# mandyxmq/NeuralBTF-tiny-cuda-nn

Hardware: AMD Instinct MI355X
Metric: training steps/sec at batch=2^18, config_hash.json (HashGrid+64-wide MLP) (higher is better)
Workload: dtype fp16 storage / fp32 MFMA accumulate; 1 GPU; HashGrid L16 F2 log2T15 s1.5 base16 + FullyFusedMLP W64 H2 ReLU, RelativeL2, Adam, B=2^18; global_batch=262144, per_gpu_batch=262144, parallelism=dp1

## Files before the change

neuralbtf-tiny-cuda-nn_amd/csrc/capi.cpp:

```cpp
#include "../../include/tcnn_mi355x.h"
#include "debug_api.h"
#include "debug_grid_bwd.h"

#include <algorithm>
#include <cmath>
#include <cstring>
#include <limits>
#include <mutex>

#include "loss_device.h"
#include "loss_torch.h"
#include "optimizers.h"
#include "runtime.h"

using namespace tcnn_amd;

namespace {
thread_local std::string g_last_error;
thread_local std::string g_str;

std::mutex g_log_mutex;
tcnn_log_callback_t g_log_cb = nullptr;
void* g_log_user = nullptr;

// ... 677 lines not shown
	return guard([&] {
		t->t->require_plain_adam("The data-parallel peer exchange");
		t->t->dp_peer_attach(blobs);
	});
}
int tcnn_trainer_dp_peer_detach(tcnn_trainer* t) {
	return guard([&] { t->t->dp_peer_detach(); });
}
int tcnn_trainer_dp_peer_set_timeout(tcnn_trainer* t, double seconds) {
	return guard([&] { t->t->dp_peer_set_timeout(seconds); });
}
int tcnn_debug_peer_loopback(tcnn_trainer* t, int nranks) {
	return guard([&] {
		t->t->require_plain_adam("The data-parallel peer exchange");
		t->t->dp_peer_loopback(nranks);
	});
}
int tcnn_trainer_dp_peer_abandon(tcnn_trainer* t) {
	return guard([&] { t->t->dp_peer_abandon(); });
}
int tcnn_trainer_dp_gather_state(tcnn_trainer* t, void* stream) {
	return guard([&] { t->t->dp_gather_state((hipStream_t)stream); });
}
float tcnn_trainer_loss(tcnn_trainer* t, void* stream) {
	float v = -1.0f;
	if (guard([&] { v = t->t->loss((hipStream_t)stream); }) != 0) return -1.0f;
	return v;
}
int tcnn_trainer_loss_value(tcnn_trainer* t, void* stream, float* out) {
	return guard([&] {
// ... 101 lines not shown
	return guard([&] {
		TCNN_CHECK(name && ptr, "optimizer_buffer: null name or result pointer");
		*ptr = t->t->optimizer_buffer(name, elem_bytes);
	});
}
int tcnn_trainer_learning_rate(const tcnn_trainer* t, float* learning_rate) {
	return guard([&] {
		TCNN_CHECK(learning_rate != nullptr, "learning_rate: null result pointer");
		*learning_rate = t->t->learning_rate();
	});
}
const char* tcnn_trainer_optimizer_schedule(const tcnn_trainer* t) { return !t->t->opt ? "adam" : t->t->opt_inline ? "inline" : "staged"; }
int tcnn_trainer_set_learning_rate(tcnn_trainer* t, float learning_rate) {
	return guard([&] { t->t->set_learning_rate(learning_rate); });
}
void* tcnn_trainer_param_gradients(tcnn_trainer* t) { return t->t->g16.p; }
float* tcnn_trainer_gradients_fp32(tcnn_trainer* t) { return t->t->g32.as<float>(); }
int tcnn_trainer_optimizer_state(tcnn_trainer* t, float** m1, float** m2, uint32_t** steps) {
	if (m1) *m1 = t->t->m1.as<float>();
	if (m2) *m2 = t->t->m2.as<float>();
	if (steps) *steps = t->t->steps.as<uint32_t>();
	return 0;
}
int tcnn_trainer_set_gradient_scale(tcnn_trainer* t, float s) {
	TrainerHost& h = *t->t;
	h.grad_scale_user = s;
	h.grad_scale = s / (float)h.dp_nranks();
	return 0;
}
int tcnn_trainer_set_loss_scale(tcnn_trainer* t, float loss_scale) {
	return guard([&] {
		TCNN_CHECK(loss_scale > 0.0f && std::isfinite(loss_scale), "set_loss_scale: the loss scale must be positive and finite");
		t->t->loss_scale = loss_scale;
// ... 183 lines not shown
```

neuralbtf-tiny-cuda-nn_amd/csrc/dp.cpp:

```cpp
#include <dlfcn.h>

#include <rccl/rccl.h>

#include <cstring>
#include <mutex>

#include "runtime.h"

namespace tcnn_amd {

namespace {
struct RcclApi {
	decltype(&ncclGetUniqueId) get_unique_id = nullptr;
	decltype(&ncclCommInitRank) comm_init_rank = nullptr;
	decltype(&ncclCommDestroy) comm_destroy = nullptr;
	decltype(&ncclAllReduce) all_reduce = nullptr;
	decltype(&ncclReduceScatter) reduce_scatter = nullptr;
	decltype(&ncclAllGather) all_gather = nullptr;
	decltype(&ncclGetErrorString) error_string = nullptr;
};

const RcclApi& rccl() {
	static std::once_flag once;
	static RcclApi api;
// ... 67 lines not shown
}

static void grow_preserve(DevBuf& b, size_t bytes, size_t valid) {
	if (b.bytes >= bytes) return;
	DevBuf n;
	n.reserve(bytes);
	TCNN_HIP_CHECK(hipMemset(n.p, 0, bytes));
	if (b.p && valid) TCNN_HIP_CHECK(hipMemcpy(n.p, b.p, valid, hipMemcpyDeviceToDevice));
	std::swap(b.p, n.p);
	std::swap(b.bytes, n.bytes);
}

void TrainerHost::set_dp(DpComm* c, bool sharded) {
	TCNN_CHECK(!peer_attached, "set_dp: the trainer is attached to a peer exchange (detach it first)");
	if (dp && dp_sharded && dp_state_partial) dp_gather_state(nullptr);
	TCNN_HIP_CHECK(hipDeviceSynchronize());
	dp = c;
	dp_sharded = c && sharded;
	dp_state_partial = false;
	grad_scale = grad_scale_user / (float)dp_nranks();
	if (graph) set_graph(use_graph);
	if (!dp_sharded) return;
	const uint64_t N = (uint64_t)c->nranks;
	dp_per = (n_params + N - 1) / N;
	const size_t pad = (size_t)(dp_per * N);
	grow_preserve(w32, pad * 4, n_params * 4);
	grow_preserve(w16, pad * 2, n_params * 2);
	grow_preserve(g16, pad * 2, n_params * 2);
	grow_preserve(g32, pad * 4, n_params * 4);
	grow_preserve(m1, pad * 4, n_params * 4);
// ... 35 lines not shown
		optimizer_step_range(st, lo, hi);
		c.all_gather(w16.p, (size_t)dp_per, 2, st);
		dp_state_partial = true;
	} else {
		optimizer_step(st);
	}
	timer.mark(st, 3);
}

void TrainerHost::dp_gather_state(hipStream_t st) {
	if (peer_attached) {
		if (dp_state_partial) dp_peer_gather_state(st);
		return;
	}
	if (!dp || !dp_sharded || !dp_state_partial) return;
	for (DevBuf* b : {&w32, &m1, &m2, &steps}) dp->all_gather(b->p, (size_t)dp_per, 4, st);
	TCNN_HIP_CHECK(hipStreamSynchronize(st));
	dp_state_partial = false;
}

}
```

neuralbtf-tiny-cuda-nn_amd/csrc/dp_peer.hip:

```cpp
#include <cstdlib>
#include <cstring>
#include <vector>

#include "adam_device.h"
#include "runtime.h"

namespace tcnn_amd {

namespace {

constexpr uint32_t PEER_MAGIC = 0x50454552u;
constexpr int PEER_MAX_RANKS = 64;
constexpr int PEER_NBUF = 4;
enum PeerBuf { PB_G32 = 0, PB_W16, PB_STATE, PB_FLAGS };
enum PeerSlot { SLOT_GRAD = 0, SLOT_WEIGHTS = 1, SLOT_GATHER = 2, SLOT_DETACH = 3, SLOT_PROBE = 4 };
constexpr int PROBE_WORD = 16;

__host__ __device__ inline uint32_t probe_token(int rank) { return PEER_MAGIC ^ (0x9e3779b9u * (uint32_t)(rank + 1)); }
enum PeerCtr { CTR_STEP = 0, CTR_SYNC = 1, CTR_ERR = 2, CTR_ARRIVE = 3 };

struct PeerBlob {
	uint32_t magic, nranks, rank, device;
	uint64_t n_params, per;
	uint64_t pci;
// ... 247 lines not shown
static void grow_keep(DevBuf& b, size_t bytes, size_t valid) {
	if (b.bytes >= bytes) return;
	DevBuf n;
	n.reserve(bytes);
	TCNN_HIP_CHECK(hipMemset(n.p, 0, bytes));
	if (b.p && valid) TCNN_HIP_CHECK(hipMemcpy(n.p, b.p, valid, hipMemcpyDeviceToDevice));
	std::swap(b.p, n.p);
	std::swap(b.bytes, n.bytes);
}

void TrainerHost::dp_peer_export(int nranks, int rank, void* blob_out) {
	TCNN_CHECK(!dp, "peer exchange: detach the RCCL communicator first (set_dp(NULL))");
	TCNN_CHECK(nranks >= 1 && rank >= 0 && rank < nranks, "peer exchange: rank outside [0, nranks)");
	TCNN_CHECK(nranks <= PEER_MAX_RANKS, "peer exchange: at most 64 ranks (the ranks of one node)");
	if (peer) dp_peer_detach();
	TCNN_HIP_CHECK(hipDeviceSynchronize());
	auto pd = std::make_shared<PeerDp>();
	pd->nranks = nranks;
	pd->rank = rank;
	const uint64_t per = ((n_params + nranks - 1) / nranks + 7) / 8 * 8;
	pd->per = per;
	const size_t pad = (size_t)(per * nranks);
	grow_keep(w32, pad * 4, n_params * 4);
	grow_keep(w16, pad * 2, n_params * 2);
	grow_keep(g16, pad * 2, n_params * 2);
	grow_keep(g32, pad * 4, n_params * 4);
	grow_keep(m1, pad * 4, n_params * 4);
	grow_keep(m2, pad * 4, n_params * 4);
	grow_keep(steps, pad * 4, n_params * 4);
	const size_t xbytes[PEER_NBUF] = {pad * 4, pad * 2, 4 * pad * 4, 256};
// ... 218 lines not shown
```

neuralbtf-tiny-cuda-nn_amd/csrc/kernels.h:

```cpp
#pragma once

#include "common.h"

namespace tcnn_amd {

struct LevelInfo;

struct GridCall {
	uint32_t D, F, L;
	HashType hash;
	bool hash_grid;
	Interp interp;
	const LevelInfo* levels;
	GridOpts opts;
};

struct GridSlice {
	uint32_t level;
	uint32_t begin;
	uint32_t end;
	uint32_t f0;
	uint32_t nf;
};

// ... 42 lines not shown
}

struct AdamArgs {
	uint32_t n, n_matrix;
	float loss_scale, grad_scale;
	float lr, beta1, beta2, eps, l2_reg, rel_decay, abs_decay, clip, nonmat_lr_factor;
	float lower_lr_bound, upper_lr_bound;
	int opt_matrix, opt_nonmatrix;
	float inv_loss_scale;
	uint32_t begin;
	const float* part;
	uint32_t n_parts, part_stride;
	const float* factor_table;
	uint32_t factor_n;
	const GridSlabMap* part_map;
};

struct AdamBuffers {
	float* w32;
	_Float16* w16;
	float* g32;
	_Float16* g16;
	float* m1;
	float* m2;
	uint32_t* steps;
};

struct GradFinalize {
	void* out = nullptr;
	float s = 1.0f;
	int out_f32 = 0;
// ... 116 lines not shown
	int dldenc_pairs;
	float* wgrad_partial;
	float* loss_partial;
};
void launch_mlp_tile_train(hipStream_t st, uint32_t W, uint32_t IN, uint32_t NH, int act, TileTrainArgs a);
bool tile_infer_supported(uint32_t W, uint32_t IN, uint32_t NH, uint32_t outp, int act);
uint32_t tile_infer_blocks(uint32_t B, uint32_t W, uint32_t IN, uint32_t NH);
void launch_mlp_tile_infer(hipStream_t st, uint32_t W, uint32_t IN, uint32_t NH, int act, int out_act, uint32_t B, const void* params16,
                           const void* enc16, void* out16);

void launch_generate_uniform(hipStream_t st, uint64_t n, uint64_t state, uint64_t inc, float* out, float lo, float hi);
void launch_generate_logistic(hipStream_t st, uint64_t n, uint64_t state, uint64_t inc, float* out, float mean, float stddev);
void launch_add_perturbation(hipStream_t st, uint32_t n, const void* out16, const float* noise, void* pert16);
void launch_adam(hipStream_t st, const AdamArgs& a, float* w32, void* w16, const float* grad32, void* grad16,
                 float* m1, float* m2, uint32_t* steps);

void launch_cast_f32_f16(hipStream_t st, const float* in, void* out, size_t n);
void launch_cast_f16_f32(hipStream_t st, const void* in, float* out, size_t n);
void launch_scale_f16(hipStream_t st, const void* in, void* out, float s, size_t n);
void launch_div_f32(hipStream_t st, float* x, float s, size_t n);
void launch_scale_f32(hipStream_t st, const float* in, float* out, float s, size_t n);
void launch_div_f16(hipStream_t st, const void* in, void* out, float s, size_t n, bool out_f32);
void launch_grad_finalize(hipStream_t st, const float* g, void* out, float s, size_t n, bool out_f32);

void launch_relative_l2(hipStream_t st, uint32_t B, uint32_t stride, uint32_t dims, float loss_scale,
                        const void* pred16, const float* target, float* values, void* grads16);

void launch_sum(hipStream_t st, const float* in, uint32_t n, float* out);

bool layered_width_supported(uint32_t w);
// ... 81 lines not shown
```

neuralbtf-tiny-cuda-nn_amd/csrc/kernels.hip:

```cpp
#include "kernels.h"

#include <cstdlib>

#include "adam_device.h"
#include "grid_device.h"
#include "mlp_fused.h"

namespace tcnn_amd {

__global__ __launch_bounds__(256) void k_reduce_groups(const float* __restrict__ in, uint32_t n_parts, uint32_t group,
                                                        uint32_t stride, uint32_t n, float* __restrict__ out, uint32_t out_stride) {
	const uint32_t p4 = (blockIdx.x * blockDim.x + threadIdx.x) * 4;
	if (p4 >= n) return;
	const uint32_t j0 = blockIdx.y * group;
	const uint32_t j1 = min(n_parts, j0 + group);
	float* dst = out + (size_t)blockIdx.y * out_stride;
	if (p4 + 4 <= n && (stride % 4) == 0 && (out_stride % 4) == 0) {
		f4 s = {0.0f, 0.0f, 0.0f, 0.0f};
		s = slab_sum((const f4*)(in + (size_t)j0 * stride + p4), stride / 4, j1 - j0);
		*(f4*)(dst + p4) = s;
	} else {
		for (uint32_t p = p4; p < n && p < p4 + 4; ++p) {
			float s = 0.0f;
			s = slab_sum(in + (size_t)j0 * stride + p, stride, j1 - j0);
// ... 137 lines not shown
}
void launch_add_perturbation(hipStream_t st, uint32_t n, const void* out16, const float* noise, void* pert16) {
	if (!n) return;
	hipLaunchKernelGGL(k_add_perturbation, dim3(div_round_up(n, 256u)), dim3(256), 0, st, n, (const _Float16*)out16, noise, (_Float16*)pert16);
	TCNN_HIP_CHECK(hipGetLastError());
}

void launch_generate_uniform(hipStream_t st, uint64_t n, uint64_t state, uint64_t inc, float* out, float lo, float hi) {
	if (n == 0) return;
	const uint64_t n_thr = (n + 3) / 4;
	hipLaunchKernelGGL(k_generate_uniform, dim3((uint32_t)((n_thr + 127) / 128)), dim3(128), 0, st, n, state, inc, out, lo, hi - lo);
	TCNN_HIP_CHECK(hipGetLastError());
}


__global__ __launch_bounds__(256) void k_adam(const AdamArgs a, float* __restrict__ w32, _Float16* __restrict__ w16,
                                               const float* __restrict__ grad32, _Float16* __restrict__ grad16,
                                               float* __restrict__ m1, float* __restrict__ m2, uint32_t* __restrict__ steps) {
	const uint32_t i = a.begin + blockIdx.x * blockDim.x + threadIdx.x;
	if (i >= a.n) return;
	float gsum;
	if (a.part) {
		const uint32_t q = a.part_map ? grid_slab_index(a.part_map, i - a.begin) : i - a.begin;
		gsum = slab_sum(a.part + q, a.part_stride, a.n_parts);
		((float*)grad32)[i] = gsum;
	} else {
		gsum = grad32[i];
	}
	const AdamBuffers s{w32, w16, (float*)grad32, grad16, m1, m2, steps};
	adam_update(a, s, i, gsum);
}

void launch_adam(hipStream_t st, const AdamArgs& a, float* w32, void* w16, const float* grad32, void* grad16,
                 float* m1, float* m2, uint32_t* steps) {
	if (a.n <= a.begin) return;
	hipLaunchKernelGGL(k_adam, dim3(div_round_up(a.n - a.begin, 256)), dim3(256), 0, st, a, w32, (_Float16*)w16, grad32, (_Float16*)grad16, m1, m2, steps);
	TCNN_HIP_CHECK(hipGetLastError());
}

__global__ void k_cast_f32_f16(const float* __restrict__ in, _Float16* __restrict__ out, size_t n) {
	const size_t i = (size_t)blockIdx.x * blockDim.x + threadIdx.x;
	if (i < n) out[i] = (_Float16)in[i];
}
__global__ void k_cast_f16_f32(const _Float16* __restrict__ in, float* __restrict__ out, size_t n) {
	const size_t i = (size_t)blockIdx.x * blockDim.x + threadIdx.x;
	if (i < n) out[i] = (float)in[i];
}
__global__ void k_scale_f16(const _Float16* __restrict__ in, _Float16* __restrict__ out, float s, size_t n) {
	const size_t i = (size_t)blockIdx.x * blockDim.x + threadIdx.x;
	if (i < n) out[i] = f16_rn((float)in[i] * s);
}
// ... 149 lines not shown
```

neuralbtf-tiny-cuda-nn_amd/csrc/runtime.cpp:

```cpp
#include "runtime.h"
#include "loss_device.h"

#include <algorithm>
#include <cctype>
#include <cmath>
#include <cstring>
#include <limits>
#include <random>

namespace tcnn_amd {

static constexpr uint64_t PCG32_MULT = 0x5851f42d4c957f2dULL;

void Pcg32::seed(uint64_t initstate, uint64_t initseq) {
	state = 0u;
	inc = (initseq << 1u) | 1u;
	next_uint();
	state += initstate;
	next_uint();
}

uint32_t Pcg32::next_uint() {
	uint64_t old = state;
	state = old * PCG32_MULT + inc;
// ... 63 lines not shown
	EngineSwitches s;
	auto on = [](const char* n) { return std::getenv(n) != nullptr; };
	s.no_fused_grid = on("TCNN_NO_FUSED_GRID");
	s.no_tile_engine = on("TCNN_NO_TILE_ENGINE");
	s.no_inrange_index = on("TCNN_NO_INRANGE_INDEX");
	s.no_forward_keep = on("TCNN_NO_FORWARD_KEEP");
	s.split_forward = on("TCNN_SPLIT_FORWARD");
	const char* bin = std::getenv("TCNN_GRID_BIN");
	s.grid_bin_all = bin && std::string(bin) == "all";
	if (const char* e = std::getenv("TCNN_GRID_BWD_CHUNKS"))
		if (std::atoi(e) > 0) s.grid_bwd_chunks = (uint32_t)std::atoi(e);
	if (const char* e = std::getenv("TCNN_GRID_BWD_RANGES"))
		if (std::atoi(e) > 0) s.grid_bwd_ranges = (uint32_t)std::atoi(e);
	if (const char* e = std::getenv("TCNN_GRID_BWD_STREAM")) s.no_grid_bwd_stream = std::string(e) == "0";
	if (const char* e = std::getenv("TCNN_WT_STORES")) s.wt_stores = (uint32_t)std::strtoul(e, nullptr, 0) & WT_STORES_ALL;
	if (const char* e = std::getenv("TCNN_GRID_BWD_PLAN")) s.grid_bwd_plan = std::string(e) == "feature" ? 1 : (std::string(e) == "range" ? 0 : -1);
	return s;
}

bool ieq(const std::string& a, const std::string& b) {
	if (a.size() != b.size()) return false;
	for (size_t i = 0; i < a.size(); ++i)
		if (std::tolower((unsigned char)a[i]) != std::tolower((unsigned char)b[i])) return false;
	return true;
}

static const struct { const char* name; uint32_t type; } k_loss_otypes[] = {
	{"L2", LOSS_L2},
	{"RelativeL2", LOSS_RELATIVE_L2},
	{"RelativeL2Luminance", LOSS_RELATIVE_L2_LUMINANCE},
// ... 1287 lines not shown
	w32.reserve(n_params * 4);
	w16.reserve(n_params * 2);
	g16.reserve(n_params * 2);
	g32.reserve(n_params * 4);
	m1.reserve(n_params * 4);
	m2.reserve(n_params * 4);
	steps.reserve(n_params * 4);
	d_loss.reserve(16);
	TCNN_HIP_CHECK(hipMemcpy(w32.p, host.data(), n_params * 4, hipMemcpyHostToDevice));
	TCNN_HIP_CHECK(hipMemset(g16.p, 0, n_params * 2));
	TCNN_HIP_CHECK(hipMemset(g32.p, 0, n_params * 4));
	TCNN_HIP_CHECK(hipMemset(m1.p, 0, n_params * 4));
	TCNN_HIP_CHECK(hipMemset(m2.p, 0, n_params * 4));
	TCNN_HIP_CHECK(hipMemset(steps.p, 0, n_params * 4));
	TCNN_HIP_CHECK(hipMemset(d_loss.p, 0, 16));
	launch_cast_f32_f16(nullptr, w32.as<float>(), w16.p, n_params);
	TCNN_HIP_CHECK(hipDeviceSynchronize());
	adam_step = 0;
	ws.wimage_valid = false;
	if (this->opt) {
		opt_allocate();
		opt_reset_weights();
		TCNN_HIP_CHECK(hipDeviceSynchronize());
	}
}

void TrainerHost::set_params_full_precision(const float* host, uint64_t n) {
	TCNN_CHECK(n == n_params, "Can't set fp params because buffer has the wrong size.");
	TCNN_HIP_CHECK(hipDeviceSynchronize());
	TCNN_HIP_CHECK(hipMemcpy(w32.p, host, n * 4, hipMemcpyHostToDevice));
	launch_cast_f32_f16(nullptr, w32.as<float>(), w16.p, n_params);
	ws.wimage_valid = false;
	TCNN_HIP_CHECK(hipDeviceSynchronize());
	opt_reset_weights();
}

void TrainerHost::training_step(hipStream_t st, uint32_t B, const float* input, const float* target, bool run_optimizer) {
	TCNN_CHECK(B % BATCH_GRANULARITY == 0, "training_step: batch size must be a multiple of 256");
	if (timer.enabled) {
		timer.sampling = (timer.counter++ % timer.every) == 0;
		if (timer.sampling) timer.marks.push_back({-1, -1, -1, -1, -1});
	}
	if (run_optimizer && use_graph && !opt && !(timer.enabled && timer.sampling) && !adam.adabound &&
	    training_step_graph(st, B, input, target))
		return;
	if (run_optimizer && opt) {
		opt_training_step(st, B, input, target);
		return;
	}
	if (run_optimizer) step_eager(st, B, input, target);
	else gradient_pass(st, B, input, target);
}

// ... 61 lines not shown
	if (run_optimizer) {
		GridAccAdam ga{};
		ga.a = adam_args_table(st, adam_step);
		ga.buf = ep.buf;
		ga.param_base = (uint32_t)n_mlp;
		ga.write_grad32 = 0;
		g.backward_acc(st, ws.gbw, B, ws.dLdenc.p, 0, 0, g32.as<float>() + n_mlp, &ga);
		timer.mark(st, 2);
		AdamArgs ag = adam_args_table(st, adam_step);
		ag.n = (uint32_t)n_mlp + g.n_lds_params;
		ag.begin = (uint32_t)n_mlp;
		ag.part = ws.gbw.partial.as<float>();
		ag.n_parts = ws.gbw.n_chunks;
		ag.part_stride = g.n_lds_params;
		ag.part_map = g.slab_map(ws.gbw.plan);
		if (!g.plans[0].slices.empty())
			launch_adam(st, ag, w32.as<float>(), w16.p, g32.as<float>(), g16.p, m1.as<float>(), m2.as<float>(), steps.as<uint32_t>());
	} else {
		g.backward_acc(st, ws.gbw, B, ws.dLdenc.p, 0, 0, gsum + n_mlp);
		timer.mark(st, 2);
		g.reduce_items(st, ws.gbw, gsum + n_mlp);
	}
	timer.mark(st, 3);
	last_B = B;
}

struct TrainerHost::StepGraph {
	static constexpr size_t MAX_GRAPHS = 8;
	hipStream_t cs = nullptr;
	hipEvent_t e0 = nullptr, e1 = nullptr;
	std::vector<std::pair<std::vector<uint64_t>, hipGraphExec_t>> execs;
	StepGraph() {
// ... 32 lines not shown
}

std::vector<uint64_t> TrainerHost::graph_key(uint32_t B, const float* input, const float* target) const {
	std::vector<uint64_t> k = {B, (uint64_t)(uintptr_t)input, (uint64_t)(uintptr_t)target, (uint64_t)ftable_valid,
	                           (uint64_t)(uintptr_t)w32.p, (uint64_t)(uintptr_t)w16.p, (uint64_t)(uintptr_t)g16.p,
	                           (uint64_t)(uintptr_t)g32.p, (uint64_t)(uintptr_t)m1.p, (uint64_t)(uintptr_t)m2.p,
	                           (uint64_t)(uintptr_t)steps.p, (uint64_t)(uintptr_t)d_loss.p, (uint64_t)(uintptr_t)d_ftable.p,
	                           (uint64_t)(uintptr_t)ws.dLdenc.p, (uint64_t)(uintptr_t)ws.dy_bound.p, (uint64_t)(uintptr_t)ws.wgrad_partial.p,
	                           (uint64_t)(uintptr_t)ws.loss_partial.p, (uint64_t)(uintptr_t)ws.wimage.p,
	                           (uint64_t)(uintptr_t)ws.gbw.partial.p, (uint64_t)(uintptr_t)ws.gbw.recs.p,
	                           (uint64_t)(uintptr_t)ws.gbw.dir.p, (uint64_t)(uintptr_t)ws.gbw.dysum.p, ws.n_fused_blocks,
	                           ws.gbw.n_chunks, (uint64_t)overlapped_ok(), (uint64_t)(uintptr_t)dp, (uint64_t)dp_sharded, dp_per,
	                           (uint64_t)(uintptr_t)ws.enc16.p, (uint64_t)(uintptr_t)ws.acts.p, (uint64_t)(uintptr_t)ws.delta0.p,
	                           (uint64_t)(uintptr_t)ws.delta1.p, (uint64_t)(uintptr_t)ws.dout16.p, (uint64_t)(uintptr_t)ws.out16.p,
	                           (uint64_t)(uintptr_t)ws.red_tmp.p, (uint64_t)(uintptr_t)ws.tile_wT.p, (uint64_t)(uintptr_t)ws.loss_sum.p,
	                           ws.n_loss_partials, (uint64_t)(uintptr_t)peer.get(), (uint64_t)peer_attached};
	const AdamArgs a = adam_args();
	const size_t n = sizeof(AdamArgs) / 8 + 1;
	std::vector<uint64_t> ab(n, 0);
	std::memcpy(ab.data(), &a, sizeof(AdamArgs));
	k.insert(k.end(), ab.begin(), ab.end());
	const GridOpts o = model->grid ? model->grid->opts() : GridOpts{};
	uint32_t ml = 0;
	std::memcpy(&ml, &o.max_level, 4);
	k.insert(k.end(), {(uint64_t)ml, (uint64_t)(uintptr_t)o.max_level_gpu, o.stochastic, o.n_features, o.active, o.inrange_index});
	uint32_t ls = 0, gs = 0;
	std::memcpy(&ls, &loss_scale, 4);
	std::memcpy(&gs, &grad_scale, 4);
	k.insert(k.end(), {(uint64_t)ls, (uint64_t)gs});
	return k;
}
// ... 6 lines not shown
		(void)adam_args_table(st, GRAPH_STEPS, GRAPH_STEPS);
	if (!graph) graph = std::make_unique<StepGraph>();
	std::vector<uint64_t> key = graph_key(B, input, target);
	hipGraphExec_t exec = graph->find(key);
	if (!exec) {
		step_eager(st, B, input, target);
		key = graph_key(B, input, target);
		TCNN_HIP_CHECK(hipStreamSynchronize(st));
		TCNN_HIP_CHECK(hipStreamSynchronize(graph->cs));
		if (graph->execs.size() >= StepGraph::MAX_GRAPHS) {
			(void)hipGraphExecDestroy(graph->execs.front().second);
			graph->execs.erase(graph->execs.begin());
		}
		const uint32_t step0 = adam_step, ftv0 = ftable_valid, lb0 = last_B;
		const bool wv0 = ws.wimage_valid, dps0 = dp_state_partial;
		hipGraph_t g = nullptr;
		const bool tim = timer.enabled;
		timer.enabled = false;
		TCNN_HIP_CHECK(hipStreamBeginCapture(graph->cs, hipStreamCaptureModeThreadLocal));
		step_eager(graph->cs, B, input, target);
		TCNN_HIP_CHECK(hipStreamEndCapture(graph->cs, &g));
		timer.enabled = tim;
		adam_step = step0;
		ftable_valid = ftv0;
		last_B = lb0;
		ws.wimage_valid = wv0;
		dp_state_partial = dps0;
		hipGraphExec_t e = nullptr;
		const hipError_t err = hipGraphInstantiate(&e, g, nullptr, nullptr, 0);
		(void)hipGraphDestroy(g);
		TCNN_HIP_CHECK(err);
		graph->execs.emplace_back(key, e);
		++graph_captures;
		return true;
	}
	TCNN_HIP_CHECK(hipGraphLaunch(exec, st));
	++adam_step;
	ws.wimage_valid = image_step;
	if ((dp && dp_sharded) || peer_attached) dp_state_partial = true;
	last_B = B;
	++graph_replays;
	return true;
}

hipEvent_t PhaseTimer::get() {
	if (next == pool.size()) {
		hipEvent_t e;
		TCNN_HIP_CHECK(hipEventCreate(&e));
		pool.push_back(e);
	}
	return pool[next++];
}

PhaseTimer::~PhaseTimer() {
// ... 47 lines not shown
	a.upper_lr_bound = std::numeric_limits<float>::max();
	if (adam.adabound) {
		a.lower_lr_bound = 0.1f - 0.1f / ((1 - adam.beta2) * (float)adam_step + 1);
		a.upper_lr_bound = 0.1f + 0.1f / ((1 - adam.beta2) * (float)adam_step);
	}
	a.opt_matrix = adam.optimize_matrix_params;
	a.opt_nonmatrix = adam.optimize_non_matrix_params;
	int e = 0;
	a.inv_loss_scale = (std::frexp(loss_scale, &e) == 0.5f) ? 1.0f / loss_scale : 0.0f;
	return a;
}

void TrainerHost::training_step_part(hipStream_t st, uint32_t B, const float* input, const float* target, int part) {
	TCNN_CHECK(B % BATCH_GRANULARITY == 0, "training_step: batch size must be a multiple of 256");
	TCNN_CHECK(part == 0 || part == 1, "training_step_part: part must be 0 or 1");
	if (!overlapped_ok()) {
		if (part == 0) training_step(st, B, input, target, false);
		return;
	}
	TCNN_CHECK(part == 0 || last_B == B, "training_step_part: part 1 must follow part 0 of the same batch");
	fused_gradient_half(st, B, input, target, part);
}

void TrainerHost::fused_gradient_half(hipStream_t st, uint32_t B, const float* input, const float* target, int half) {
	NetworkHost& m = *model;
	float* g = g32.as<float>();
	if (half == 0) {
		m.fused_kernel(st, ws, loss_pass(B, input, target, g), false, true);
		launch_column_sums(st, ws.wgrad_partial.as<float>(), ws.n_fused_blocks, (uint32_t)n_mlp, g);
		launch_sum(st, ws.loss_partial.as<float>(), ws.n_loss_partials, d_loss.as<float>());
// ... 22 lines not shown
		const uint32_t ahead = std::min(ftable_cap, (std::max(upto, reserve) + 1023u) / 1024u * 1024u);
		h_ftable.resize(ahead);
		for (uint32_t t = ftable_valid + 1; t <= ahead; ++t)
			h_ftable[t - 1] = std::sqrt(1.0f - std::pow(adam.beta2, (float)t)) / (1.0f - std::pow(adam.beta1, (float)t));
		TCNN_HIP_CHECK(hipMemcpyAsync(d_ftable.as<float>() + ftable_valid, h_ftable.data() + ftable_valid, (size_t)(ahead - ftable_valid) * 4,
		                              hipMemcpyHostToDevice, st));
		TCNN_HIP_CHECK(hipStreamSynchronize(st));
		ftable_valid = ahead;
	}
	a.factor_table = d_ftable.as<float>();
	a.factor_n = ftable_valid;
	return a;
}

void TrainerHost::optimizer_step(hipStream_t st) {
	if (opt) {
		launch_grad_f16(st, g32.as<float>(), g16.p, grad_scale, n_params);
		OptStep s;
		s.st = st;
		s.g32 = g32.as<float>();
		s.gscale = grad_scale;
		s.g16 = g16.p;
		opt_step(*opt, s);
		return;
	}
	adam_apply(st, g32.as<float>(), grad_scale, g16.p);
}

std::unique_ptr<TrainerFwdCtx> TrainerHost::forward(hipStream_t st, uint32_t B, const float* input, const float* target, const float* pdf,
                                                    const void* ext_dLdy16, bool prep_dinput, const float* perturbation,
                                                    bool use_inference_params) {
	TCNN_CHECK(B % BATCH_GRANULARITY == 0, "forward: batch size must be a multiple of 256");
	TCNN_CHECK(ext_dLdy16 || target, "forward: a target (or an external dL/dy) is required");
	NetworkHost& m = *model;
	const uint32_t OUTP = m.mlp.padded_output;
	auto c = std::make_unique<TrainerFwdCtx>();
	c->B = B;
	c->out16.reserve((size_t)B * OUTP * 2);
	const void* params16 = use_inference_params ? params_inference() : w16.p;
	c->inference_params = params16 != w16.p;
	c->layout = m.forward_keep(st, ws, B, input, params16, c->out16.p, prep_dinput, c->keep);
// ... 6 lines not shown
		const void* loss_in = c->out16.p;
		if (perturbation) {
			c->pert16.reserve((size_t)B * OUTP * 2);
			launch_add_perturbation(st, B * OUTP, c->out16.p, perturbation, c->pert16.p);
			loss_in = c->pert16.p;
		}
		launch_relative_l2_partial(st, B, OUTP, n_output_dims, loss_scale, loss_in, target, c->dLdy16.p, c->lpart.as<float>(),
		                           m.loss_type, pdf);
	}
	ws.wimage_valid = false;
	return c;
}

void TrainerHost::backward(hipStream_t st, const TrainerFwdCtx& c, uint32_t B, const float* input, float* dL_dinput, int gradient_mode) {
	TCNN_CHECK(B == c.B, "backward: batch size differs from the forward's");
	TCNN_CHECK(!c.inference_params,
	           "backward: use_inference_params is honoured by inference and by a forward without a backward only; this context's "
	           "forward read the optimizer's custom weights, and gradients are taken at the training parameters");
	float* dst = g32.as<float>();
	if (gradient_mode != 0) {
		g32_acc.reserve(n_params * 4);
		dst = g32_acc.as<float>();
	}
	TrainPass p;
	p.B = B;
	p.pos = input;
	p.params16 = w16.p;
	p.dims = n_output_dims;
	p.dout16 = c.dLdy();
	p.grad32 = dst;
// ... 2 lines not shown
	p.kept_layout = c.layout;
	model->fwd_bwd(st, ws, p);
	if (gradient_mode == 1) launch_add_f32(st, dst, g32.as<float>(), n_params);
	ws.wimage_valid = false;
	last_B = B;
}

float TrainerHost::ctx_loss(hipStream_t st, const TrainerFwdCtx& c) {
	if (c.ext) return 0.0f;
	launch_sum(st, c.lpart.as<float>(), c.n_lpart, d_loss.as<float>());
	return loss(st);
}

void TrainerHost::optimizer_step_range(hipStream_t st, uint64_t begin, uint64_t end) {
	require_plain_adam("optimizer_step_range");
	TCNN_CHECK(begin <= end && end <= n_params, "optimizer_step_range: range outside the parameter vector");
	++adam_step;
	AdamArgs a = adam_args_table(st, adam_step);
	a.begin = (uint32_t)begin;
	a.n = (uint32_t)end;
	launch_adam(st, a, w32.as<float>(), w16.p, g32.as<float>(), g16.p, m1.as<float>(), m2.as<float>(), steps.as<uint32_t>());
	ws.wimage_valid = false;
}

float TrainerHost::loss(hipStream_t st) {
	float v = 0.0f;
	TCNN_HIP_CHECK(hipMemcpyAsync(&v, d_loss.p, 4, hipMemcpyDeviceToHost, st));
	TCNN_HIP_CHECK(hipStreamSynchronize(st));
	return v;
}
// ... 11 lines not shown
```

neuralbtf-tiny-cuda-nn_amd/csrc/runtime.h:

```cpp
#pragma once

#include <json.hpp>

#include <array>
#include <cstdlib>
#include <memory>
#include <string>
#include <vector>

#include "common.h"
#include "grid_device.h"
#include "kernels.h"
#include "optimizer_tree.h"
#include "wt_store.h"

namespace tcnn_amd {

using json = nlohmann::json;

struct Pcg32 {
	uint64_t state = 0x853c49e6748fea9bULL, inc = 0xda3e39cb94b95bdbULL;
	Pcg32() = default;
	explicit Pcg32(uint64_t initstate, uint64_t initseq = 1u) { seed(initstate, initseq); }
	void seed(uint64_t initstate, uint64_t initseq = 1u);
// ... 36 lines not shown
};
enum : int { PLAN_RANGE = 0, PLAN_FEATURE = 1 };

struct EngineSwitches {
	bool no_fused_grid = false;
	bool no_tile_engine = false;
	bool no_inrange_index = false;
	bool no_forward_keep = false;
	bool split_forward = false;
	bool grid_bin_all = false;
	uint32_t grid_bwd_chunks = 0;
	uint32_t grid_bwd_ranges = 0;
	int grid_bwd_plan = -1;
	bool no_grid_bwd_stream = false;
	uint32_t wt_stores = WT_STORES_DEFAULT;
	static EngineSwitches from_env();
};

struct GridEncodingHost {
	EngineSwitches sw = EngineSwitches::from_env();
	GridDesc desc{};
	uint32_t n_features = 0;
	uint32_t n_to_pad = 0;
	uint32_t n_params = 0;
	bool stochastic = false;
	float max_level = 1000.0f;
	const float* max_level_gpu = nullptr;
	std::vector<LevelInfo> levels;
	GridPlan plans[2];
	uint32_t first_binned = 0;
// ... 332 lines not shown
	AdamHost adam;
	std::string loss_otype;
	uint64_t n_params = 0, n_mlp = 0;
	DevBuf w32, w16, g16, g32, m1, m2, steps, d_loss;
	DevBuf d_ftable;
	std::vector<float> h_ftable;
	uint32_t ftable_cap = 0, ftable_valid = 0;
	float ftable_b1 = 0.0f, ftable_b2 = 0.0f;
	AdamArgs adam_args_table(hipStream_t st, uint32_t upto, uint32_t reserve = 0);
	StepWorkspace ws;
	uint32_t adam_step = 0;
	float grad_scale = 1.0f;
	float grad_scale_user = 1.0f;
	float loss_scale = 128.0f;
	uint32_t last_B = 0;
	bool overlapped_ok() const { return model->fused_ok(); }
	void training_step_overlapped(hipStream_t st, uint32_t B, const float* input, const float* target, bool run_optimizer,
	                              float* grad_out = nullptr);
	void training_step_sequential(hipStream_t st, uint32_t B, const float* input, const float* target, bool run_optimizer,
	                              float* grad_out = nullptr);
	TrainPass loss_pass(uint32_t B, const float* input, const float* target, float* grad32) const;
	void gradient_pass(hipStream_t st, uint32_t B, const float* input, const float* target, float* grad_out = nullptr);
	void fused_gradient_half(hipStream_t st, uint32_t B, const float* input, const float* target, int half);
	void step_adam(hipStream_t st, uint32_t B, const float* input, const float* target);
	AdamArgs adam_args() const;

	std::unique_ptr<OptNode> opt;
	bool opt_inline = false;
	struct OptStep {
		hipStream_t st = nullptr;
// ... 87 lines not shown
```

neuralbtf-tiny-cuda-nn_amd/csrc/snapshot.cpp:

```cpp
#include <cmath>
#include <cstring>
#include <functional>
#include <map>
#include <string>
#include <vector>

#include "runtime.h"

namespace tcnn_amd {
namespace {

struct MsgWriter {
	std::vector<uint8_t> b;
	void u8(uint8_t v) { b.push_back(v); }
	void be(uint64_t v, int n) {
		for (int i = n - 1; i >= 0; --i) b.push_back((uint8_t)(v >> (8 * i)));
	}
	void map(uint32_t n) {
		if (n <= 15) u8((uint8_t)(0x80 | n));
		else if (n <= 0xffff) { u8(0xde); be(n, 2); }
		else { u8(0xdf); be(n, 4); }
	}
	void str(const std::string& s) {
		const size_t n = s.size();
// ... 208 lines not shown
	return json();
}

}

std::string TrainerHost::serialize_json(bool with_optimizer) {
	const std::vector<uint8_t> b = serialize(with_optimizer);
	MsgReader r{b.data(), b.data() + b.size()};
	return to_json(r.value()).dump();
}

std::vector<uint8_t> TrainerHost::serialize(bool with_optimizer) {
	TCNN_CHECK(!(with_optimizer && dp_sharded && dp_state_partial),
	           "serialize(optimizer): the sharded data-parallel optimizer state is current only on each rank's shard; "
	           "gather it first (tcnn_trainer_dp_gather_state)");
	TCNN_HIP_CHECK(hipDeviceSynchronize());
	const size_t n = n_params;
	MsgWriter w;
	w.map(with_optimizer ? 4 : 3);
	w.str("n_params");
	w.uint(n);
	std::function<void(const OptNode*)> write_opt = [&](const OptNode* node) {
		auto bin = [&](const char* key, const DevBuf& b, size_t bytes) {
			const auto h = d2h(b, bytes);
			w.str(key);
			w.bin(h.data(), h.size());
		};
		if (!node || node->kind == OptKind::Adam) {
			w.map(5);
			w.str("base_learning_rate");
// ... 42 lines not shown
	};
	if (with_optimizer) {
		w.str("optimizer");
		write_opt(opt.get());
	}
	std::vector<uint8_t> ph(n * 2);
	if (n) TCNN_HIP_CHECK(hipMemcpy(ph.data(), params_inference(), n * 2, hipMemcpyDeviceToHost));
	w.str("params_binary");
	w.bin(ph.data(), ph.size());
	w.str("params_type");
	w.str("__half");
	return std::move(w.b);
}

void TrainerHost::deserialize(const void* data, size_t size) {
	TCNN_HIP_CHECK(hipDeviceSynchronize());
	MsgValue root;
	if (size > 0 && ((const char*)data)[0] == '{') {
		root = from_json_text(json::parse(std::string((const char*)data, size)));
	} else {
		MsgReader r{(const uint8_t*)data, (const uint8_t*)data + size};
		root = r.value();
	}
	TCNN_CHECK(root.kind == MsgValue::Map, "snapshot: top level must be a map");
	const size_t n = n_params;
	const std::string type = root.has("params_type") ? root.at("params_type").s : "__half";
	const MsgValue& pb = root.at("params_binary");
	if (type == "float") {
		const std::string b = bin_of(pb, n * 4, "params_binary");
		std::vector<float> host(n);
// ... 63 lines not shown
```

Before: 12430 training steps/s (2^18-sample batches, whole job).

## Skip per-step grid gradient stores in fused Adam and defer materialization lazily

The fused Adam kernel for the hash-grid slab gradients gains lean variants. By default it no longer writes the reduced fp32/fp16 gradients on every step, and an optional mode keeps one step counter per 256-parameter block instead of per-parameter step counts. Consumers that read gradients or optimizer state (C API getters, serialize, DP attach, optimizer_step, backward) first call lean_settle, which runs a separate kernel to materialize the gradients or expand the step counts. This saves memory write bandwidth in the hot optimizer kernel, at the cost of extra state tracking and a risk of stale data on any path that misses a settle call.

```diff
diff --git a/neuralbtf-tiny-cuda-nn_amd/csrc/capi.cpp b/neuralbtf-tiny-cuda-nn_amd/csrc/capi.cpp
--- a/neuralbtf-tiny-cuda-nn_amd/csrc/capi.cpp
+++ b/neuralbtf-tiny-cuda-nn_amd/csrc/capi.cpp
@@ -1,5 +1,6 @@
 #include "../../include/tcnn_mi355x.h"
 #include "debug_api.h"
+#include "debug_adam.h"
 #include "debug_grid_bwd.h"
 
 #include <algorithm>
@@ -715,6 +716,12 @@
 	return guard([&] {
 		t->t->require_plain_adam("The data-parallel peer exchange");
 		t->t->dp_peer_loopback(nranks);
+	});
+}
+int tcnn_debug_adam_uniform_blocks(tcnn_trainer* t, uint32_t* n_uniform, uint32_t* n_blocks) {
+	return guard([&] {
+		if (n_blocks) *n_blocks = t->t->n_step_blocks();
+		if (n_uniform) *n_uniform = t->t->uniform_step_blocks();
 	});
 }
 int tcnn_trainer_dp_peer_abandon(tcnn_trainer* t) {
@@ -846,9 +853,16 @@
 int tcnn_trainer_set_learning_rate(tcnn_trainer* t, float learning_rate) {
 	return guard([&] { t->t->set_learning_rate(learning_rate); });
 }
-void* tcnn_trainer_param_gradients(tcnn_trainer* t) { return t->t->g16.p; }
-float* tcnn_trainer_gradients_fp32(tcnn_trainer* t) { return t->t->g32.as<float>(); }
+void* tcnn_trainer_param_gradients(tcnn_trainer* t) {
+	if (guard([&] { t->t->lean_settle(TrainerHost::LeanUse::Caller); }) != 0) return nullptr;
+	return t->t->g16.p;
+}
+float* tcnn_trainer_gradients_fp32(tcnn_trainer* t) {
+	if (guard([&] { t->t->lean_settle(TrainerHost::LeanUse::Caller); }) != 0) return nullptr;
+	return t->t->g32.as<float>();
+}
 int tcnn_trainer_optimizer_state(tcnn_trainer* t, float** m1, float** m2, uint32_t** steps) {
+	if (int rc = guard([&] { t->t->lean_settle(TrainerHost::LeanUse::Caller); })) return rc;
 	if (m1) *m1 = t->t->m1.as<float>();
 	if (m2) *m2 = t->t->m2.as<float>();
 	if (steps) *steps = t->t->steps.as<uint32_t>();
diff --git a/neuralbtf-tiny-cuda-nn_amd/csrc/debug_adam.h b/neuralbtf-tiny-cuda-nn_amd/csrc/debug_adam.h
--- /dev/null
+++ b/neuralbtf-tiny-cuda-nn_amd/csrc/debug_adam.h
@@ -0,0 +1,13 @@
+#ifndef TCNN_DEBUG_ADAM_H
+#define TCNN_DEBUG_ADAM_H
+#include "../../include/tcnn_mi355x.h"
+#ifdef __cplusplus
+extern "C" {
+#endif
+
+int tcnn_debug_adam_uniform_blocks(tcnn_trainer* t, uint32_t* n_uniform, uint32_t* n_blocks);
+
+#ifdef __cplusplus
+}
+#endif
+#endif
diff --git a/neuralbtf-tiny-cuda-nn_amd/csrc/dp.cpp b/neuralbtf-tiny-cuda-nn_amd/csrc/dp.cpp
--- a/neuralbtf-tiny-cuda-nn_amd/csrc/dp.cpp
+++ b/neuralbtf-tiny-cuda-nn_amd/csrc/dp.cpp
@@ -105,6 +105,7 @@
 void TrainerHost::set_dp(DpComm* c, bool sharded) {
 	TCNN_CHECK(!peer_attached, "set_dp: the trainer is attached to a peer exchange (detach it first)");
 	if (dp && dp_sharded && dp_state_partial) dp_gather_state(nullptr);
+	lean_settle(c ? LeanUse::Caller : LeanUse::Write);
 	TCNN_HIP_CHECK(hipDeviceSynchronize());
 	dp = c;
 	dp_sharded = c && sharded;
@@ -170,6 +171,7 @@
 		return;
 	}
 	if (!dp || !dp_sharded || !dp_state_partial) return;
+	lean_settle(LeanUse::Write);
 	for (DevBuf* b : {&w32, &m1, &m2, &steps}) dp->all_gather(b->p, (size_t)dp_per, 4, st);
 	TCNN_HIP_CHECK(hipStreamSynchronize(st));
 	dp_state_partial = false;
diff --git a/neuralbtf-tiny-cuda-nn_amd/csrc/dp_peer.hip b/neuralbtf-tiny-cuda-nn_amd/csrc/dp_peer.hip
--- a/neuralbtf-tiny-cuda-nn_amd/csrc/dp_peer.hip
+++ b/neuralbtf-tiny-cuda-nn_amd/csrc/dp_peer.hip
@@ -285,6 +285,7 @@
 	TCNN_CHECK(nranks >= 1 && rank >= 0 && rank < nranks, "peer exchange: rank outside [0, nranks)");
 	TCNN_CHECK(nranks <= PEER_MAX_RANKS, "peer exchange: at most 64 ranks (the ranks of one node)");
 	if (peer) dp_peer_detach();
+	lean_settle(LeanUse::Caller);
 	TCNN_HIP_CHECK(hipDeviceSynchronize());
 	auto pd = std::make_shared<PeerDp>();
 	pd->nranks = nranks;
diff --git a/neuralbtf-tiny-cuda-nn_amd/csrc/kernels.h b/neuralbtf-tiny-cuda-nn_amd/csrc/kernels.h
--- a/neuralbtf-tiny-cuda-nn_amd/csrc/kernels.h
+++ b/neuralbtf-tiny-cuda-nn_amd/csrc/kernels.h
@@ -80,7 +80,13 @@
 	const float* factor_table;
 	uint32_t factor_n;
 	const GridSlabMap* part_map;
-};
+	uint32_t lean;
+	uint32_t* step_blocks;
+};
+
+enum : uint32_t { ADAM_LEAN_GRADS = 1u, ADAM_LEAN_STEPS = 2u, ADAM_LEAN_ALL = 3u, ADAM_LEAN_DEFAULT = ADAM_LEAN_GRADS };
+constexpr uint32_t ADAM_STEPS_DIVERGED = 0xFFFFFFFFu;
+constexpr uint32_t ADAM_STEP_BLOCK = 256;
 
 struct AdamBuffers {
 	float* w32;
@@ -227,6 +233,9 @@
 void launch_add_perturbation(hipStream_t st, uint32_t n, const void* out16, const float* noise, void* pert16);
 void launch_adam(hipStream_t st, const AdamArgs& a, float* w32, void* w16, const float* grad32, void* grad16,
                  float* m1, float* m2, uint32_t* steps);
+void launch_grid_slab_gradients(hipStream_t st, const float* in, uint32_t n_parts, uint32_t stride, uint32_t n, const GridSlabMap* map,
+                                float grad_scale, float* grad32, void* grad16);
+void launch_adam_steps_expand(hipStream_t st, const uint32_t* step_blocks, uint32_t n, uint32_t* steps);
 
 void launch_cast_f32_f16(hipStream_t st, const float* in, void* out, size_t n);
 void launch_cast_f16_f32(hipStream_t st, const void* in, float* out, size_t n);
diff --git a/neuralbtf-tiny-cuda-nn_amd/csrc/kernels.hip b/neuralbtf-tiny-cuda-nn_amd/csrc/kernels.hip
--- a/neuralbtf-tiny-cuda-nn_amd/csrc/kernels.hip
+++ b/neuralbtf-tiny-cuda-nn_amd/csrc/kernels.hip
@@ -175,27 +175,125 @@
 }
 
 
+template <uint32_t LEAN>
 __global__ __launch_bounds__(256) void k_adam(const AdamArgs a, float* __restrict__ w32, _Float16* __restrict__ w16,
                                                const float* __restrict__ grad32, _Float16* __restrict__ grad16,
                                                float* __restrict__ m1, float* __restrict__ m2, uint32_t* __restrict__ steps) {
+	static_assert(ADAM_STEP_BLOCK == 256, "one step-count word per workgroup");
 	const uint32_t i = a.begin + blockIdx.x * blockDim.x + threadIdx.x;
-	if (i >= a.n) return;
-	float gsum;
-	if (a.part) {
-		const uint32_t q = a.part_map ? grid_slab_index(a.part_map, i - a.begin) : i - a.begin;
-		gsum = slab_sum(a.part + q, a.part_stride, a.n_parts);
-		((float*)grad32)[i] = gsum;
+	if constexpr (LEAN == 0) {
+		if (i >= a.n) return;
+		float gsum;
+		if (a.part) {
+			const uint32_t q = a.part_map ? grid_slab_index(a.part_map, i - a.begin) : i - a.begin;
+			gsum = slab_sum(a.part + q, a.part_stride, a.n_parts);
+			((float*)grad32)[i] = gsum;
+		} else {
+			gsum = grad32[i];
+		}
+		const AdamBuffers s{w32, w16, (float*)grad32, grad16, m1, m2, steps};
+		adam_update(a, s, i, gsum);
 	} else {
-		gsum = grad32[i];
-	}
-	const AdamBuffers s{w32, w16, (float*)grad32, grad16, m1, m2, steps};
-	adam_update(a, s, i, gsum);
+		constexpr bool GRADS = (LEAN & ADAM_LEAN_GRADS) == 0, BLOCKS = (LEAN & ADAM_LEAN_STEPS) != 0;
+		const bool live = i < a.n;
+		if (!BLOCKS && !live) return;
+		uint32_t word = ADAM_STEPS_DIVERGED;
+		if (BLOCKS) word = a.step_blocks[blockIdx.x];
+		float gsum = 0.0f, w = 0.0f, mo1 = 0.0f, mo2 = 0.0f;
+		if (live) {
+			const uint32_t q = a.part_map ? grid_slab_index(a.part_map, i - a.begin) : i - a.begin;
+			gsum = slab_sum(a.part + q, a.part_stride, a.n_parts);
+			w = w32[i];
+			mo1 = m1[i];
+			mo2 = m2[i];
+		}
+		const bool uniform = word != ADAM_STEPS_DIVERGED;
+		uint32_t step = uniform ? word : (live ? steps[i] : 0u);
+		bool upd = false;
+		if (live) {
+			_Float16 g16;
+			upd = adam_core(a, i, gsum, g16, w, mo1, mo2, step);
+			if (GRADS) {
+				((float*)grad32)[i] = gsum;
+				if (grad16) grad16[i] = g16;
+			}
+			if (upd) {
+				w32[i] = w;
+				m1[i] = mo1;
+				m2[i] = mo2;
+				w16[i] = f16_rn(w);
+			}
+		}
+		if (!BLOCKS) {
+			if (upd) steps[i] = step;
+			return;
+		}
+		if (uniform) {
+			const uint32_t n_live = min(ADAM_STEP_BLOCK, a.n - (a.begin + blockIdx.x * ADAM_STEP_BLOCK));
+			const uint32_t n_upd = (uint32_t)__syncthreads_count(upd ? 1 : 0);
+			if (n_upd == n_live) {
+				if (threadIdx.x == 0) a.step_blocks[blockIdx.x] = word + 1u;
+			} else if (n_upd != 0) {
+				if (live) steps[i] = step;
+				if (threadIdx.x == 0) a.step_blocks[blockIdx.x] = ADAM_STEPS_DIVERGED;
+			}
+		} else {
+			if (upd) steps[i] = step;
+			__shared__ uint32_t first;
+			if (threadIdx.x == 0) first = step;
+			__syncthreads();
+			const uint32_t f = first;
+			const int same = __syncthreads_and((!live || step == f) ? 1 : 0);
+			if (same && threadIdx.x == 0 && f != ADAM_STEPS_DIVERGED) a.step_blocks[blockIdx.x] = f;
+		}
+	}
 }
 
 void launch_adam(hipStream_t st, const AdamArgs& a, float* w32, void* w16, const float* grad32, void* grad16,
                  float* m1, float* m2, uint32_t* steps) {
 	if (a.n <= a.begin) return;
-	hipLaunchKernelGGL(k_adam, dim3(div_round_up(a.n - a.begin, 256)), dim3(256), 0, st, a, w32, (_Float16*)w16, grad32, (_Float16*)grad16, m1, m2, steps);
+	const dim3 grid(div_round_up(a.n - a.begin, ADAM_STEP_BLOCK));
+	const uint32_t lean = a.part ? (a.lean & ADAM_LEAN_ALL) : 0u;
+	TCNN_CHECK(!(lean & ADAM_LEAN_STEPS) || a.step_blocks, "launch_adam: block step counts without their buffer");
+#define TCNN_LAUNCH_ADAM(L) \
+	hipLaunchKernelGGL(k_adam<L>, grid, dim3(256), 0, st, a, w32, (_Float16*)w16, grad32, (_Float16*)grad16, m1, m2, steps)
+	switch (lean) {
+		case 0: TCNN_LAUNCH_ADAM(0u); break;
+		case 1: TCNN_LAUNCH_ADAM(1u); break;
+		case 2: TCNN_LAUNCH_ADAM(2u); break;
+		default: TCNN_LAUNCH_ADAM(3u); break;
+	}
+#undef TCNN_LAUNCH_ADAM
+	TCNN_HIP_CHECK(hipGetLastError());
+}
+
+__global__ __launch_bounds__(256) void k_grid_slab_gradients(const float* __restrict__ in, uint32_t n_parts, uint32_t stride, uint32_t n,
+                                                              const GridSlabMap* __restrict__ map, float grad_scale,
+                                                              float* __restrict__ grad32, _Float16* __restrict__ grad16) {
+	const uint32_t p = blockIdx.x * blockDim.x + threadIdx.x;
+	if (p >= n) return;
+	const float s = slab_sum(in + (map ? grid_slab_index(map, p) : p), stride, n_parts);
+	grad32[p] = s;
+	grad16[p] = f16_rn(s * grad_scale);
+}
+
+void launch_grid_slab_gradients(hipStream_t st, const float* in, uint32_t n_parts, uint32_t stride, uint32_t n, const GridSlabMap* map,
+                                float grad_scale, float* grad32, void* grad16) {
+	if (!n) return;
+	hipLaunchKernelGGL(k_grid_slab_gradients, dim3(div_round_up(n, 256)), dim3(256), 0, st, in, n_parts, stride, n, map, grad_scale, grad32,
+	                   (_Float16*)grad16);
+	TCNN_HIP_CHECK(hipGetLastError());
+}
+
+__global__ __launch_bounds__(256) void k_adam_steps_expand(const uint32_t* __restrict__ step_blocks, uint32_t n, uint32_t* __restrict__ steps) {
+	const uint32_t word = step_blocks[blockIdx.x];
+	const uint32_t i = blockIdx.x * ADAM_STEP_BLOCK + threadIdx.x;
+	if (word != ADAM_STEPS_DIVERGED && i < n) steps[i] = word;
+}
+
+void launch_adam_steps_expand(hipStream_t st, const uint32_t* step_blocks, uint32_t n, uint32_t* steps) {
+	if (!n) return;
+	hipLaunchKernelGGL(k_adam_steps_expand, dim3(div_round_up(n, ADAM_STEP_BLOCK)), dim3(256), 0, st, step_blocks, n, steps);
 	TCNN_HIP_CHECK(hipGetLastError());
 }
 
diff --git a/neuralbtf-tiny-cuda-nn_amd/csrc/runtime.cpp b/neuralbtf-tiny-cuda-nn_amd/csrc/runtime.cpp
--- a/neuralbtf-tiny-cuda-nn_amd/csrc/runtime.cpp
+++ b/neuralbtf-tiny-cuda-nn_amd/csrc/runtime.cpp
@@ -101,6 +101,7 @@
 		if (std::atoi(e) > 0) s.grid_bwd_ranges = (uint32_t)std::atoi(e);
 	if (const char* e = std::getenv("TCNN_GRID_BWD_STREAM")) s.no_grid_bwd_stream = std::string(e) == "0";
 	if (const char* e = std::getenv("TCNN_WT_STORES")) s.wt_stores = (uint32_t)std::strtoul(e, nullptr, 0) & WT_STORES_ALL;
+	if (const char* e = std::getenv("TCNN_ADAM_LEAN")) s.adam_lean = (uint32_t)std::strtoul(e, nullptr, 0) & ADAM_LEAN_ALL;
 	if (const char* e = std::getenv("TCNN_GRID_BWD_PLAN")) s.grid_bwd_plan = std::string(e) == "feature" ? 1 : (std::string(e) == "range" ? 0 : -1);
 	return s;
 }
@@ -1418,6 +1419,13 @@
 	TCNN_HIP_CHECK(hipMemset(m2.p, 0, n_params * 4));
 	TCNN_HIP_CHECK(hipMemset(steps.p, 0, n_params * 4));
 	TCNN_HIP_CHECK(hipMemset(d_loss.p, 0, 16));
+	if (n_step_blocks()) {
+		step_blocks.reserve((size_t)n_step_blocks() * 4);
+		TCNN_HIP_CHECK(hipMemset(step_blocks.p, 0, (size_t)n_step_blocks() * 4));
+	}
+	grads_stale = false;
+	steps_current = true;
+	step_blocks_diverged = false;
 	launch_cast_f32_f16(nullptr, w32.as<float>(), w16.p, n_params);
 	TCNN_HIP_CHECK(hipDeviceSynchronize());
 	adam_step = 0;
@@ -1441,6 +1449,7 @@
 
 void TrainerHost::training_step(hipStream_t st, uint32_t B, const float* input, const float* target, bool run_optimizer) {
 	TCNN_CHECK(B % BATCH_GRANULARITY == 0, "training_step: batch size must be a multiple of 256");
+	if (!(run_optimizer && lean_mask() != 0)) lean_settle(LeanUse::Write);
 	if (timer.enabled) {
 		timer.sampling = (timer.counter++ % timer.every) == 0;
 		if (timer.sampling) timer.marks.push_back({-1, -1, -1, -1, -1});
@@ -1532,8 +1541,12 @@
 		ag.n_parts = ws.gbw.n_chunks;
 		ag.part_stride = g.n_lds_params;
 		ag.part_map = g.slab_map(ws.gbw.plan);
+		ag.lean = lean_mask();
+		ag.step_blocks = step_blocks.as<uint32_t>();
+		TCNN_CHECK(steps_current || (ag.lean & ADAM_LEAN_STEPS), "training step: block step counts were not expanded");
 		if (!g.plans[0].slices.empty())
 			launch_adam(st, ag, w32.as<float>(), w16.p, g32.as<float>(), g16.p, m1.as<float>(), m2.as<float>(), steps.as<uint32_t>());
+		lean_note_step(st, ag.lean);
 	} else {
 		g.backward_acc(st, ws.gbw, B, ws.dLdenc.p, 0, 0, gsum + n_mlp);
 		timer.mark(st, 2);
@@ -1596,7 +1609,8 @@
 	                           (uint64_t)(uintptr_t)ws.enc16.p, (uint64_t)(uintptr_t)ws.acts.p, (uint64_t)(uintptr_t)ws.delta0.p,
 	                           (uint64_t)(uintptr_t)ws.delta1.p, (uint64_t)(uintptr_t)ws.dout16.p, (uint64_t)(uintptr_t)ws.out16.p,
 	                           (uint64_t)(uintptr_t)ws.red_tmp.p, (uint64_t)(uintptr_t)ws.tile_wT.p, (uint64_t)(uintptr_t)ws.loss_sum.p,
-	                           ws.n_loss_partials, (uint64_t)(uintptr_t)peer.get(), (uint64_t)peer_attached};
+	                           ws.n_loss_partials, (uint64_t)(uintptr_t)peer.get(), (uint64_t)peer_attached,
+	                           (uint64_t)lean_mask(), (uint64_t)(uintptr_t)step_blocks.p};
 	const AdamArgs a = adam_args();
 	const size_t n = sizeof(AdamArgs) / 8 + 1;
 	std::vector<uint64_t> ab(n, 0);
@@ -1633,6 +1647,9 @@
 		}
 		const uint32_t step0 = adam_step, ftv0 = ftable_valid, lb0 = last_B;
 		const bool wv0 = ws.wimage_valid, dps0 = dp_state_partial;
+		const bool gst0 = grads_stale, sc0 = steps_current, sbd0 = step_blocks_diverged;
+		const float sgs0 = stale_grad_scale;
+		hipStream_t const lst0 = lean_st;
 		hipGraph_t g = nullptr;
 		const bool tim = timer.enabled;
 		timer.enabled = false;
@@ -1645,6 +1662,11 @@
 		last_B = lb0;
 		ws.wimage_valid = wv0;
 		dp_state_partial = dps0;
+		grads_stale = gst0;
+		steps_current = sc0;
+		step_blocks_diverged = sbd0;
+		stale_grad_scale = sgs0;
+		lean_st = lst0;
 		hipGraphExec_t e = nullptr;
 		const hipError_t err = hipGraphInstantiate(&e, g, nullptr, nullptr, 0);
 		(void)hipGraphDestroy(g);
@@ -1657,6 +1679,7 @@
 	++adam_step;
 	ws.wimage_valid = image_step;
 	if ((dp && dp_sharded) || peer_attached) dp_state_partial = true;
+	if (image_step) lean_note_step(st, lean_mask());
 	last_B = B;
 	++graph_replays;
 	return true;
@@ -1734,6 +1757,7 @@
 void TrainerHost::training_step_part(hipStream_t st, uint32_t B, const float* input, const float* target, int part) {
 	TCNN_CHECK(B % BATCH_GRANULARITY == 0, "training_step: batch size must be a multiple of 256");
 	TCNN_CHECK(part == 0 || part == 1, "training_step_part: part must be 0 or 1");
+	lean_settle(LeanUse::Write);
 	if (!overlapped_ok()) {
 		if (part == 0) training_step(st, B, input, target, false);
 		return;
@@ -1786,6 +1810,7 @@
 }
 
 void TrainerHost::optimizer_step(hipStream_t st) {
+	lean_settle(LeanUse::Write);
 	if (opt) {
 		launch_grad_f16(st, g32.as<float>(), g16.p, grad_scale, n_params);
 		OptStep s;
@@ -1797,6 +1822,65 @@
 		return;
 	}
 	adam_apply(st, g32.as<float>(), grad_scale, g16.p);
+}
+
+uint32_t TrainerHost::n_step_blocks() const {
+	return model->grid ? div_round_up(model->grid->n_lds_params, ADAM_STEP_BLOCK) : 0u;
+}
+
+uint32_t TrainerHost::lean_mask() const {
+	if (opt || dp || peer_attached || !overlapped_ok() || !model->grid || model->grid->plans[0].slices.empty()) return 0;
+	uint32_t m = adam_lean;
+	if (grads_eager) m &= ~ADAM_LEAN_GRADS;
+	if (steps_per_param) m &= ~ADAM_LEAN_STEPS;
+	return m;
+}
+
+void TrainerHost::lean_note_step(hipStream_t st, uint32_t lean) {
+	lean_st = st;
+	grads_stale = (lean & ADAM_LEAN_GRADS) != 0;
+	stale_grad_scale = grad_scale;
+	if (lean & ADAM_LEAN_STEPS) {
+		steps_current = false;
+		step_blocks_diverged = false;
+	}
+}
+
+void TrainerHost::grads_materialize() {
+	if (!grads_stale) return;
+	const GridEncodingHost& g = *model->grid;
+	launch_grid_slab_gradients(lean_st, ws.gbw.partial.as<float>(), ws.gbw.n_chunks, g.n_lds_params, g.n_lds_params, g.slab_map(ws.gbw.plan),
+	                           stale_grad_scale, g32.as<float>() + n_mlp, g16.as<_Float16>() + n_mlp);
+	grads_stale = false;
+}
+
+void TrainerHost::steps_expand(LeanUse use) {
+	if (!n_step_blocks()) return;
+	if (!steps_current) {
+		launch_adam_steps_expand(lean_st, step_blocks.as<uint32_t>(), model->grid->n_lds_params, steps.as<uint32_t>() + n_mlp);
+		steps_current = true;
+	}
+	if (use != LeanUse::Read && !step_blocks_diverged) {
+		TCNN_HIP_CHECK(hipMemsetAsync(step_blocks.p, 0xFF, (size_t)n_step_blocks() * 4, lean_st));
+		step_blocks_diverged = true;
+	}
+}
+
+void TrainerHost::lean_settle(LeanUse use) {
+	grads_materialize();
+	steps_expand(use);
+	if (use == LeanUse::Caller) grads_eager = steps_per_param = true;
+}
+
+uint32_t TrainerHost::uniform_step_blocks() {
+	const uint32_t n = n_step_blocks();
+	if (!n) return 0;
+	std::vector<uint32_t> h(n);
+	TCNN_HIP_CHECK(hipStreamSynchronize(lean_st));
+	TCNN_HIP_CHECK(hipMemcpy(h.data(), step_blocks.p, (size_t)n * 4, hipMemcpyDeviceToHost));
+	uint32_t u = 0;
+	for (uint32_t w : h) u += w != ADAM_STEPS_DIVERGED ? 1u : 0u;
+	return u;
 }
 
 std::unique_ptr<TrainerFwdCtx> TrainerHost::forward(hipStream_t st, uint32_t B, const float* input, const float* target, const float* pdf,
@@ -1833,6 +1917,7 @@
 
 void TrainerHost::backward(hipStream_t st, const TrainerFwdCtx& c, uint32_t B, const float* input, float* dL_dinput, int gradient_mode) {
 	TCNN_CHECK(B == c.B, "backward: batch size differs from the forward's");
+	lean_settle(LeanUse::Write);
 	TCNN_CHECK(!c.inference_params,
 	           "backward: use_inference_params is honoured by inference and by a forward without a backward only; this context's "
 	           "forward read the optimizer's custom weights, and gradients are taken at the training parameters");
@@ -1865,6 +1950,7 @@
 
 void TrainerHost::optimizer_step_range(hipStream_t st, uint64_t begin, uint64_t end) {
 	require_plain_adam("optimizer_step_range");
+	lean_settle(LeanUse::Write);
 	TCNN_CHECK(begin <= end && end <= n_params, "optimizer_step_range: range outside the parameter vector");
 	++adam_step;
 	AdamArgs a = adam_args_table(st, adam_step);
diff --git a/neuralbtf-tiny-cuda-nn_amd/csrc/runtime.h b/neuralbtf-tiny-cuda-nn_amd/csrc/runtime.h
--- a/neuralbtf-tiny-cuda-nn_amd/csrc/runtime.h
+++ b/neuralbtf-tiny-cuda-nn_amd/csrc/runtime.h
@@ -74,6 +74,7 @@
 	int grid_bwd_plan = -1;
 	bool no_grid_bwd_stream = false;
 	uint32_t wt_stores = WT_STORES_DEFAULT;
+	uint32_t adam_lean = ADAM_LEAN_DEFAULT;
 	static EngineSwitches from_env();
 };
 
@@ -436,6 +437,24 @@
 	float grad_scale_user = 1.0f;
 	float loss_scale = 128.0f;
 	uint32_t last_B = 0;
+
+	uint32_t adam_lean = EngineSwitches::from_env().adam_lean;
+	bool grads_eager = false, steps_per_param = false;
+	bool grads_stale = false;
+	float stale_grad_scale = 1.0f;
+	hipStream_t lean_st = nullptr;
+	DevBuf step_blocks;
+	bool steps_current = true;
+	bool step_blocks_diverged = false;
+	uint32_t n_step_blocks() const;
+	uint32_t lean_mask() const;
+	enum class LeanUse { Read, Write, Caller };
+	void lean_settle(LeanUse use);
+	void grads_materialize();
+	void steps_expand(LeanUse use);
+	void lean_note_step(hipStream_t st, uint32_t lean);
+	uint32_t uniform_step_blocks();
+
 	bool overlapped_ok() const { return model->fused_ok(); }
 	void training_step_overlapped(hipStream_t st, uint32_t B, const float* input, const float* target, bool run_optimizer,
 	                              float* grad_out = nullptr);
diff --git a/neuralbtf-tiny-cuda-nn_amd/csrc/snapshot.cpp b/neuralbtf-tiny-cuda-nn_amd/csrc/snapshot.cpp
--- a/neuralbtf-tiny-cuda-nn_amd/csrc/snapshot.cpp
+++ b/neuralbtf-tiny-cuda-nn_amd/csrc/snapshot.cpp
@@ -246,6 +246,7 @@
 	TCNN_CHECK(!(with_optimizer && dp_sharded && dp_state_partial),
 	           "serialize(optimizer): the sharded data-parallel optimizer state is current only on each rank's shard; "
 	           "gather it first (tcnn_trainer_dp_gather_state)");
+	lean_settle(LeanUse::Read);
 	TCNN_HIP_CHECK(hipDeviceSynchronize());
 	const size_t n = n_params;
 	MsgWriter w;
@@ -318,6 +319,7 @@
 }
 
 void TrainerHost::deserialize(const void* data, size_t size) {
+	lean_settle(LeanUse::Write);
 	TCNN_HIP_CHECK(hipDeviceSynchronize());
 	MsgValue root;
 	if (size > 0 && ((const char*)data)[0] == '{') {
```

Result: faster. 12560 training steps/s (2^18-sample batches, whole job) (median of 6 runs) (+1.0%).
